# TheMTank/GridUniverse

Measured on AMD Instinct MI355X. Metric: env-steps/sec at N_envs on 32×32 grid, 1/2/4/8 MI355X; bit-exact vs CPU, higher is better.
Workload: dtype int32; 1 GPU; c3: 65536 envs per GPU on the 32x32 generator maze (random.seed(123); np.random.seed(123)), uniform device-RNG actions, auto-reset, 1000 env-steps per launch, int32 (obs,reward,done) rows; envs_per_gpu=65536, env_steps_per_launch=1000, global_envs=65536, parallelism=env-index shards, no data-path collective

## Files before the change

### griduniverse_amd/_lib.py

```python
import ctypes
import os
import re
import subprocess

import numpy as np

_HERE = os.path.dirname(os.path.abspath(__file__))
LIB_PATH = os.environ.get('GU_LIB_PATH') or os.path.join(_HERE, 'lib', 'libgu.so')
CSRC = os.path.join(_HERE, 'csrc')

GU_OK = 0
ERR_NAMES = {-1: 'GU_ERR_INVALID', -2: 'GU_ERR_HIP', -3: 'GU_ERR_NOMEM', -4: 'GU_ERR_STATE',
             -5: 'GU_ERR_COMM', -6: 'GU_ERR_UNSUPPORTED'}

F_AUTO_RESET, F_TRAJECTORY, F_STATS, F_PINNED_IO, F_PACKED = 1, 2, 4, 8, 16
POLICY_UNIFORM, POLICY_STREAM, POLICY_GREEDY, POLICY_SAMPLE = 0, 1, 2, 3
TD_Q_LEARNING, TD_SARSA = 0, 1
NSTEP_MAX = 16
LAMBDA_MAX = 64
REINFORCE_MAX = 1024
IS_MAX = 1024
SEARCH_MAX_M = 64
SEARCH_MAX_D = 256
EXPLORE_MAX_C = 4096
# ... 70 lines not shown
    'gu_read_stats': [_vp, _vp, _vp],
    'gu_get_state': [_vp, _vp, _vp, _vp, _vp],
    'gu_set_state': [_vp, _vp, _vp, _vp, _vp],
    'gu_get_stores': [_vp, _i32, _vp, _vp],
    'gu_done_indices': [_vp, _vp, _vp],
    'gu_look_step_ahead': [_vp, _i64, _vp, _vp, _i32, _vp, _vp, _vp],
    'gu_td_init': [_vp, _f64],
    'gu_td_run': [_vp, _i64, _i32, _f64, _f64, _u32, _u32],
    'gu_td_get_q': [_vp, _i64, _i64, _vp],
    'gu_td_set_q': [_vp, _i64, _i64, _vp],
    'gu_esarsa_run': [_vp, _i64, _f64, _f64, _u32, _u32],
    'gu_double_init': [_vp, _f64],
    'gu_double_run': [_vp, _i64, _f64, _f64, _u32, _u32],
    'gu_double_get_q': [_vp, _i64, _i64, _vp],
    'gu_double_set_q': [_vp, _i64, _i64, _vp],
    'gu_dyna_init': [_vp],
    'gu_dyna_run': [_vp, _i64, _i32, _f64, _f64, _u32, _u32],
    'gu_dyna_get_model': [_vp, _i64, _i64, _vp, _vp, _vp, _vp, _vp],
    'gu_sweep_init': [_vp],
    'gu_sweep_run': [_vp, _i64, _i32, _f64, _f64, _f64, _u32, _u32],
    'gu_sweep_get_queue': [_vp, _i64, _i64, _vp, _vp],
    'gu_diag_sweep_heap': [_vp, _i64, _i64, _vp, _vp],
    'gu_diag_rollout_form': [_vp, _vp, _i32, _vp],
    'gu_search_run': [_vp, _i64, _i32, _i32, _f64, _f64, _u32, _u32, _u32],
    'gu_search_get': [_vp, _i64, _i64, _vp, _vp],
    'gu_explore_init': [_vp],
    'gu_explore_set_tables': [_vp, _i32, _vp, _vp],
    'gu_explore_run': [_vp, _i64, _i32, _f64, _f64, _u32, _u32],
    'gu_explore_get_counts': [_vp, _i64, _i64, _vp],
    'gu_explore_set_counts': [_vp, _i64, _i64, _vp],
    'gu_mcts_init': [_vp, _i32],
    'gu_mcts_set_tables': [_vp, _i32, _vp, _vp, _vp],
    'gu_mcts_run': [_vp, _i64, _i32, _i32, _i32, _f64, _f64, _u32, _u32, _u32],
    'gu_mcts_get': [_vp, _i64, _i64, _vp, _vp, _vp, _vp],
    'gu_mcts_get_tree': [_vp, _i64, _i64, _vp, _vp, _vp, _vp, _vp, _vp],
    'gu_nstep_run': [_vp, _i64, _i32, _i32, _f64, _f64, _u32, _u32],
    'gu_nstep_get_window': [_vp, _i64, _i64, _vp, _vp, _vp],
    'gu_lambda_run': [_vp, _i64, _i32, _i32, _f64, _f64, _f64, _u32, _u32],
    'gu_lambda_get_window': [_vp, _i64, _i64, _vp],
    'gu_ac_init': [_vp, _f64, _f64],
    'gu_ac_run': [_vp, _i64, _f64, _f64, _f64, _u32],
    'gu_ac_get': [_vp, _i64, _i64, _vp, _vp],
    'gu_ac_set': [_vp, _i64, _i64, _vp, _vp],
    'gu_reinforce_run': [_vp, _i64, _i32, _f64, _f64, _f64, _u32],
    'gu_reinforce_get_episode': [_vp, _i64, _i64, _vp, _vp, _vp],
    'gu_is_init': [_vp],
# ... 188 lines not shown
```

### griduniverse_amd/csrc/gu_internal.hpp

```cpp
#pragma once
#include <hip/hip_runtime.h>
#include <stdint.h>
#include <atomic>
#include <string>
#include <vector>

#include "../../include/gu.h"
#include "../../include/gu_diag.h"

#define GU_CELL_OPEN_MASK 0x0Fu
#define GU_CELL_TERM 0x10u
#define GU_CELL_TERM_BIT 4
#define GU_CELL_RPLUS 0x20u
#define GU_CELL_RMINUS 0x40u
#ifndef GU_WIDE_STORE_PAD
#define GU_WIDE_STORE_PAD()                         \
    do {                                            \
        __builtin_amdgcn_sched_barrier(0);          \
        asm volatile("s_nop 1" ::: "memory");       \
        __builtin_amdgcn_sched_barrier(0);          \
    } while (0)
#endif
#define GU_ACTION_OK(raw) ((uint32_t)((int32_t)(raw) + 4) < 8u)
#define GU_CELL_WALL 0x80u
// ... 90 lines not shown
    int32_t overlay_bits = 0;
    uint32_t overlay_param = 0;
    uint32_t overlay_init = 0;
    std::vector<uint8_t> box_flags;
    int32_t fruit_value[3] = {0, 0, 0};
    uint8_t *d_kind = nullptr;
    uint64_t delta_lut = 0;
    int32_t *d_starts = nullptr;
    int32_t *d_nstarts = nullptr;
    int32_t n_starts = 0;
    int32_t start0 = 0;
    int32_t max_starts = 0;
    bool all_single_start = true;
    int32_t n_grids = 1;
    int64_t group = 0;

    int32_t *d_out3 = nullptr;
    uint32_t *d_episode = nullptr;
    int32_t *d_out3_alt = nullptr;
    uint32_t *d_episode_alt = nullptr;
    uint64_t *d_done_bits_alt = nullptr;
    uint32_t *d_nib = nullptr;
    bool nib_valid = false;
    uint32_t *d_tcount = nullptr;
    uint64_t steps_taken = 0;
    int64_t off_lo = 0, off_hi = 0;
    bool off_exact = true;
    uint64_t seed = 0;
    uint32_t seed_prefix = 0;

    int32_t *d_actions = nullptr;
    uint32_t *d_actions_packed = nullptr;
    int64_t actions_T = 0;
    int64_t actions_cap = 0;

    int32_t *d_traj = nullptr;
    int64_t traj_T = 0;
    int traj_kind = 0;
    int traj_written = 0;
    int32_t traj_candidates = 0;
    float traj_probe_ms_best = 0.0f, traj_probe_ms_worst = 0.0f;
    std::vector<float> traj_probe_ms;
    std::vector<uint64_t> traj_probe_addr;
    int32_t traj_kept = -1;
    float traj_search_ms = 0.0f;
    uint64_t traj_peak_bytes = 0;
// ... 334 lines not shown
```

### griduniverse_amd/csrc/gu_kernels.hip

```cpp
#include "gu_overlay.hpp"

#include <cstdio>
#include <cstdlib>

#include <algorithm>
#include <cstring>
#include <vector>

struct ResetArgs {
    int32_t *pos, *done;
    uint32_t *episode;
    const int32_t *starts;
    const uint8_t *mask;
    const int32_t *choice;
    uint64_t *done_bits;
    uint32_t n_starts, seed_prefix, env_id0;
    int64_t N;
    int32_t only_done;
    GridSel gs;
};

__global__ void __launch_bounds__(GU_BLOCK) gu_reset_kernel(const ResetArgs a)
{
    const int64_t e = (int64_t)blockIdx.x * blockDim.x + threadIdx.x;
// ... 329 lines not shown
    pace->bar_num = (uint16_t)gu_opt(h, GU_OPT_PACE_BAR_NUM);
    pace->gain_q = (uint32_t)gu_opt(h, GU_OPT_PACE_GAIN_Q);
    pace->dec_q = (uint32_t)gu_opt(h, GU_OPT_PACE_DEC_Q);
    pace->probe_every = (uint32_t)gu_opt(h, GU_OPT_PACE_PROBE_EVERY);
    pace->adapt = (uint32_t)gu_opt(h, GU_OPT_PACE_ADAPT);
    pace->fixed = 0;
    return GU_OK;
}

int gu_pace_for(gu_engine *h, const GuRolloutPlan &p, int64_t T, GuPaceArgs *pace)
{
    *pace = GuPaceArgs{};
    const int64_t opt = gu_opt(h, GU_OPT_ROLLOUT_PACE);
    if (opt == 0) return GU_OK;
    if (p.pace_eligible && !(opt > 0 && gu_opt(h, GU_OPT_PACE_RECORD) == 0)) {
        GU_TRY(gu_pace_ring_for(h, p.pace_slot, T, p.pace_blocks, p.pace_block, p.row_bytes, pace));
        if (opt > 0) pace->period = (uint32_t)opt, pace->fixed = 1;
        return GU_OK;
    }
    if (opt > 0) pace->period = (uint32_t)opt;
    return GU_OK;
}

__global__ void __launch_bounds__(256) gu_nibble_planes_kernel(const uint8_t *__restrict__ cell, GridSel gs, int32_t W, int32_t H, int32_t dwords, int64_t N,
                                                               uint32_t *__restrict__ out)
{
    const int64_t i = (int64_t)blockIdx.x * blockDim.x + threadIdx.x;
    const int64_t total = ((N + 63) / 64) * dwords * 64;
    if (i >= total) return;
    const int64_t lane = i & 63, j = (i >> 6) % dwords, wave = (i >> 6) / dwords, e = wave * 64 + lane;
    uint32_t word = 0x88888888u;
    if (e < N) {
        const uint8_t *f = cell + (e / gs.group) * gs.grid_stride;
        word = 0;
        for (int32_t k = 0; k < 8; ++k) {
            const int32_t p = (int32_t)j * 8 + k, yp = p / (W + 1), xp = p % (W + 1);
            const bool real = yp >= 1 && yp <= H && xp >= 1;
            const uint32_t b = real ? f[(yp - 1) * W + xp - 1] : GU_CELL_WALL;
            const uint32_t four = ((b >> 5) & 3u) | (((b >> GU_CELL_TERM_BIT) & 1u) << 2) | ((b >> 7) << 3);
            word |= four << (4 * k);
        }
    }
    out[i] = word;
}

int gu_nibble_planes(gu_engine *h)
{
    if (h->nib_valid) return GU_OK;
    const int32_t dwords = gu_nibble_dwords(h);
    const int64_t total = ((h->N + 63) / 64) * dwords * 64;
    if (!h->d_nib) GU_HIP(hipMalloc((void **)&h->d_nib, (size_t)total * sizeof(uint32_t)));
    hipLaunchKernelGGL(gu_nibble_planes_kernel, dim3(gu_blocks(total, 256)), dim3(256), 0, h->stream, h->d_cell, gu_grid_sel(h), h->W, h->H, dwords, h->N, h->d_nib);
    GU_HIP(hipGetLastError());
    h->nib_valid = true;
    return GU_OK;
}

static int gu_rollout_straddles(gu_engine *h, int64_t T, int32_t policy, bool *straddle, uint32_t *epoch_lo)
{
    const bool draws = policy == GU_POLICY_UNIFORM || policy == GU_POLICY_SAMPLE;
    int64_t lo = std::max<int64_t>((int64_t)h->steps_taken + h->off_lo, 0), hi = (int64_t)h->steps_taken + h->off_hi + T - 1;
    if (draws && (lo >> 32) != (hi >> 32) && !h->off_exact) {
        std::vector<int32_t> off((size_t)h->N);
        GU_HIP(hipMemcpyAsync(off.data(), h->d_tcount, (size_t)h->N * 4, hipMemcpyDeviceToHost, h->stream));
        GU_HIP(hipStreamSynchronize(h->stream));
        const auto mm = std::minmax_element(off.begin(), off.end());
        h->off_lo = *mm.first, h->off_hi = *mm.second, h->off_exact = true;
        lo = std::max<int64_t>((int64_t)h->steps_taken + h->off_lo, 0), hi = (int64_t)h->steps_taken + h->off_hi + T - 1;
    }
    *straddle = draws && (lo >> 32) != (hi >> 32);
    *epoch_lo = (uint32_t)(lo >> 32);
    return GU_OK;
}

int gu_launch_rollout(gu_engine *h, int64_t T, int32_t policy, uint32_t flags)
{
    GU_REQUIRE(!(h->overlay && (flags & GU_F_PACKED)), GU_ERR_UNSUPPORTED, "a rollout under %s (gu_set_%s) writes int32 rows only: GU_F_PACKED is refused",
               GU_OVERLAY_NAME[h->overlay], GU_OVERLAY_NAME[h->overlay]);
    GU_REQUIRE(!h->trail_cap || (flags & (GU_F_TRAJECTORY | GU_F_PACKED)), GU_ERR_UNSUPPORTED,
// ... 10 lines not shown
    if (policy == GU_POLICY_SAMPLE)
        hipLaunchKernelGGL(gu_pi_threshold_kernel, dim3(gu_blocks(h->S, 256)), dim3(256), 0, h->stream, h->d_pi[h->vi_cur], h->S, h->d_pi_thr);
    for (bool no_pairs = false; !(p.family == GU_PLAN_KSTEP ? gu_kstep_ensure(h, p) : p.family == GU_PLAN_ROWS ? gu_rows_ensure(h, p, &no_pairs) : true);) {
        exclude |= no_pairs ? GU_PLAN_NO_PAIRS : 1u << p.family;
        p = gu_rollout_plan(h, T, policy, flags, straddle, exclude);
    }

    RolloutArgs a{};
    const int64_t rows = p.traj ? h->traj_T * h->N : 0;
    a.cell = h->d_cell, a.cell_bytes = h->cell_bytes, a.S = h->S, a.W = h->W, a.lut = h->delta_lut, a.gs = gu_grid_sel(h);
    a.greedy = h->d_greedy, a.pi_thr = h->d_pi_thr, a.actions = h->d_actions_packed;
    a.pos = h->pos(), a.reward = h->reward(), a.done = h->done(), a.episode = h->d_episode, a.tcount = h->d_tcount, a.done_bits = h->d_done_bits;
    a.starts = h->d_starts, a.n_starts = (uint32_t)h->n_starts, a.env_id0 = (uint32_t)h->env_id0;
    a.tr_obs = h->d_traj, a.tr_reward = h->d_traj ? h->d_traj + rows : nullptr, a.tr_done = h->d_traj ? h->d_traj + 2 * rows : nullptr;
    a.ret = h->d_ret, a.episodes_fin = h->d_episodes_fin;
    a.N = h->N, a.T = T, a.steps_taken = (uint32_t)h->steps_taken, a.steps_hi = (uint32_t)(h->steps_taken >> 32);
    a.straddle = straddle ? 1 : 0;
    a.seed_prefix0 = h->seed_prefix, a.seed_prefix = straddle ? h->seed_prefix : gu_rng_seed_prefix_epoch(h->seed_prefix, epoch_lo);
    a.gs.per_wave = p.per_wave, a.pi_lds = p.pi_lds, a.stream_lds_off = p.stream_lds_off, a.stream_lds_words = p.stream_lds_words;
    a.half_waves = p.half, a.entry_table = p.entry_table, a.xcd_remap = p.xcd_remap;
    if (p.family == GU_PLAN_ROWS) a.rows = p.table_policy ? h->d_prow : h->d_rows[p.which], a.rows2 = p.pair ? h->d_rows2[p.which] : nullptr, a.row_shift = p.row_shift;
    if (p.family == GU_PLAN_KSTEP) a.rows = h->d_mrows[p.which];
    if (p.need_nib) {
        a.nib = h->d_nib, a.nib_dwords = gu_nibble_dwords(h);
        const uint64_t wp = (uint64_t)(uint16_t)(int16_t)((h->W + 1) * 32), mwp = (uint64_t)(uint16_t)(int16_t)(-(h->W + 1) * 32);
        a.lut_p = mwp | (32ull << 16) | (wp << 32) | ((uint64_t)(uint16_t)(int16_t)-32 << 48);
    }
    if (p.pace_slot >= 0) GU_TRY(gu_pace_for(h, p, T, &a.pace));

    switch (p.family) {
    case GU_PLAN_WIND:
    case GU_PLAN_FRUIT:
    case GU_PLAN_DOORS:
    case GU_PLAN_BOXES: gu_overlay_launch_rollout(h, p, a); break;
    case GU_PLAN_KSTEP: gu_kstep_launch(h, p, a); break;
    case GU_PLAN_ROWS:
        if (!gu_rows_launch(h, p, a)) return gu_fail(GU_ERR_HIP, "gu_rollout_rows_kernel reports static LDS: its table must start at LDS address 0");
        break;
    default: {
        auto launch = policy == GU_POLICY_UNIFORM ? gu_rollout_uniform : policy == GU_POLICY_STREAM ? gu_rollout_stream : policy == GU_POLICY_GREEDY ? gu_rollout_greedy : gu_rollout_sample;
        if (!launch(h, p, a)) {
            p = gu_rollout_plan(h, T, policy, flags, straddle, exclude | GU_PLAN_NO_MAP5);
            a.xcd_remap = p.xcd_remap ? 1 : 0;
            launch(h, p, a);
        }
    }
    }
    GU_HIP(hipGetLastError());
    gu_rollout_plan_form(p, h->rollout_form);
// ... 87 lines not shown
```

### griduniverse_amd/csrc/gu_rollout.hpp

```cpp
#pragma once
#include "gu_map.hpp"
#include "gu_rollout_plan.hpp"

#include <cstdlib>
#include <functional>
#include <type_traits>

__device__ __forceinline__ uint32_t gu_sample_action(uint32_t word, const uint4 q)
{
    return (uint32_t)(word >= q.x) + (uint32_t)(word >= q.y) + (uint32_t)(word >= q.z) - q.w;
}


#define GU_DPP_REDUCE(x, OP)                                                                                     \
    do {                                                                                                         \
        uint32_t o_;                                                                                             \
        o_ = (uint32_t)__builtin_amdgcn_update_dpp(0, (int)(x), 0x111, 0xF, 0xF, false), (x) = OP((x), o_);      \
        o_ = (uint32_t)__builtin_amdgcn_update_dpp(0, (int)(x), 0x112, 0xF, 0xF, false), (x) = OP((x), o_);      \
        o_ = (uint32_t)__builtin_amdgcn_update_dpp(0, (int)(x), 0x114, 0xF, 0xF, false), (x) = OP((x), o_);      \
        o_ = (uint32_t)__builtin_amdgcn_update_dpp(0, (int)(x), 0x118, 0xF, 0xF, false), (x) = OP((x), o_);      \
        o_ = (uint32_t)__builtin_amdgcn_update_dpp(0, (int)(x), 0x142, 0xA, 0xF, false), (x) = OP((x), o_);      \
        o_ = (uint32_t)__builtin_amdgcn_update_dpp(0, (int)(x), 0x143, 0xC, 0xF, false), (x) = OP((x), o_);      \
    } while (0)
#define GU_OP_ADD(a_, b_) ((a_) + (b_))
// ... 282 lines not shown
            step16(word);
        }
    }
    uint32_t q = 0;
    if (TAIL16) {
        for (; i + 16 <= T; i += 16, q += 16) {
            const uint32_t sel = q >> 4;
            step16(sel == 0 ? w[0] : sel == 1 ? w[1] : w[2]);
        }
    }
    for (; i < T; ++i, ++q) {
        const uint32_t sel = q >> 4, word = sel == 0 ? w[0] : sel == 1 ? w[1] : sel == 2 ? w[2] : w[3];
        step1((word >> (2u * (q & 15u))) & 3u);
    }
}

#ifndef GU_STORE_AUX
#define GU_STORE_AUX 18
#endif
#ifndef GU_STORE_AUX_PACKED
#define GU_STORE_AUX_PACKED 16
#endif
typedef uint32_t gu_v3u __attribute__((ext_vector_type(3)));
template <int POLICY, int AUTO, int TRAJ, bool STATS, int MAP>
__global__ void __launch_bounds__(GU_MAX_BLOCK) gu_rollout_kernel(const RolloutArgs a)
{
    constexpr bool LDS = MAP == 1 || MAP == 3;
    extern __shared__ __attribute__((aligned(16))) uint8_t smem[];
    GuPacer pacer;
    pacer.fetch(a.pace, TRAJ == 1 || TRAJ == 3);
    const int64_t e64 = (int64_t)gu_env_block(a.xcd_remap) * blockDim.x + threadIdx.x;
    const bool live = e64 < a.N;
    const uint32_t e = (uint32_t)e64;
    int32_t s = 0, r = 0;
    uint32_t d = 0, ep = 0, tcount0 = 0;
    if (live) {
        s = a.pos[e];
        r = a.reward[e];
        d = (uint32_t)a.done[e];
        ep = a.episode[e];
        tcount0 = a.tcount[e];
    }
    CellMap m = gu_stage_map<LDS>(a.cell, a.cell_bytes, smem, a.gs, MAP == 3 ? 1 : 2);
    const uint32_t nib_region = MAP == 5 ? (threadIdx.x >> 6) * (uint32_t)a.nib_dwords * 256u : 0u;
    if (MAP == 5) {
        const size_t wave = ((size_t)blockIdx.x * blockDim.x + threadIdx.x) >> 6;
        const uint4 *src = reinterpret_cast<const uint4 *>(a.nib + wave * (size_t)a.nib_dwords * 64u);
        uint4 *dst = reinterpret_cast<uint4 *>(smem + nib_region);
        if (wave * 64u < (size_t)a.N)
            for (int32_t i = threadIdx.x & 63; i < a.nib_dwords * 16; i += 64) dst[i] = src[i];
        __syncthreads();
    }
    const uint8_t *greedy = a.greedy;
    if (MAP == 1 && POLICY == GU_POLICY_GREEDY) {
        uint8_t *dst = smem + 2 * a.cell_bytes;
        for (int32_t i = threadIdx.x * 16; i < a.cell_bytes; i += blockDim.x * 16)
            *reinterpret_cast<uint4 *>(dst + i) = *reinterpret_cast<const uint4 *>(a.greedy + i);
        __syncthreads();
        greedy = dst;
    }
    const bool thr_in_lds = MAP == 1 && POLICY == GU_POLICY_SAMPLE && a.pi_lds;
    uint4 *thr_lds = reinterpret_cast<uint4 *>(smem + 2 * a.cell_bytes);
    if (thr_in_lds) {
        for (int32_t i = threadIdx.x; i < a.S; i += blockDim.x) thr_lds[i] = a.pi_thr[i];
        __syncthreads();
    }
    if (!live) return;
    LaneGrid lg = gu_lane_grid<LDS>(a.gs, a.starts, a.n_starts, e, m);

    const uint32_t t_lane = tcount0 + a.steps_taken;
    const uint32_t prefix = gu_rng_prefix(a.seed_prefix, a.env_id0 + e);
    const uint32_t prefix0 = AUTO == 2 ? gu_rng_prefix(a.seed_prefix0, a.env_id0 + e) : prefix;
    const uint32_t epoch0 = (uint32_t)((uint64_t)((int64_t)(((uint64_t)a.steps_hi << 32) | a.steps_taken) + (int64_t)(int32_t)tcount0) >> 32);
    auto prefix_at = [&](uint32_t t) {
        return gu_rng_prefix(gu_rng_seed_prefix_epoch(a.seed_prefix0, epoch0 + (t < t_lane ? 1u : 0u)), a.env_id0 + e);
    };
    constexpr uint32_t TERM5 = 0x20u, TERM5_BIT = 5u;
    auto flags5 = [](uint32_t b) { return (((b >> 5) & 3u) << 3) | (((b >> GU_CELL_TERM_BIT) & 1u) << TERM5_BIT) | ((b >> 7) << 6); };
    uint32_t flags = MAP == 5 ? flags5(m.f[s]) : m.f[s];
    int32_t ret = 0, fin = 0;
    const int32_t W = a.W;
    const uint64_t lut = a.lut;
    const int32_t start0 = lg.starts[0];
    const uint32_t start0_flags = MAP == 5 ? flags5(m.f[start0]) : m.f[start0];
    auto padded = [&](int32_t c) { return (int32_t)(((uint32_t)(c + c / W + W + 2) << 5) + nib_region); };
    int32_t sq = MAP == 5 ? padded(s) : 0;
    const int32_t start0_q = MAP == 5 ? padded(start0) : 0;
    typedef __attribute__((address_space(3))) const uint32_t *lds_word_ptr;
    const uint32_t lane4 = (threadIdx.x & 63u) << 2;
    auto word_at = [&](int32_t cq) { return *(lds_word_ptr)(uintptr_t)(((uint32_t)cq & 0xFFFFFF00u) | lane4); };
    auto four_of = [](uint32_t word, int32_t cq) { return __builtin_amdgcn_ubfe(word, (uint32_t)cq >> 3, 4); };
    auto four_at = [&](int32_t cq) { return four_of(word_at(cq), cq); };
    auto cell5 = [&](int32_t cq) { return four_at(cq) << 3; };
    auto move5 = [&](uint32_t act, int32_t delta, auto &&in_the_shadow) {
        int32_t cand = s + delta;
        asm volatile("" : "+v"(cand));
        const int32_t candq = sq + gu_delta<true>(act, a.lut_p, 0);
        const uint32_t word = word_at(candq);
        in_the_shadow();
        const uint32_t four = four_of(word, candq);
        const bool go = ((flags & TERM5) | four) < 8u;
        s = go ? cand : s;
        sq = go ? candq : sq;
        flags = go ? four << 3 : flags;
    };
    char *po = (char *)a.tr_obs, *pr = (char *)a.tr_reward, *pd = (char *)a.tr_done;
    const char *pa = (const char *)a.actions;
    const uint32_t e4 = e * 4u;
    const int64_t row = a.N * 4;
    const uint32_t row32 = (uint32_t)row;
    const int64_t trow = TRAJ == 3 ? a.N * 12 : row;
    const uint32_t trow32 = (uint32_t)trow;
    const uint32_t te = TRAJ == 3 ? e * 12u : e4;
    __amdgpu_buffer_rsrc_t ro = __builtin_amdgcn_make_buffer_rsrc(po, 0, 0xFFFFFFFFu, 0x00020000);
    __amdgpu_buffer_rsrc_t rr = __builtin_amdgcn_make_buffer_rsrc(pr, 0, 0xFFFFFFFFu, 0x00020000);
    __amdgpu_buffer_rsrc_t rd = __builtin_amdgcn_make_buffer_rsrc(pd, 0, 0xFFFFFFFFu, 0x00020000);
    auto emit = [&](int32_t s_, int32_t r_, uint32_t d_, uint32_t soff) {
        if (TRAJ == 1) {
            __builtin_amdgcn_raw_buffer_store_b32(s_, ro, e4, soff, GU_STORE_AUX);
            __builtin_amdgcn_raw_buffer_store_b32(r_, rr, e4, soff, GU_STORE_AUX);
            __builtin_amdgcn_raw_buffer_store_b32((int32_t)d_, rd, e4, soff, GU_STORE_AUX);
        } else if (TRAJ == 2) {
            __builtin_amdgcn_raw_buffer_store_b32((int32_t)((uint32_t)s_ | (((uint32_t)r_ & 0xFFu) << 16) | (d_ << 24)), ro, e4, soff, GU_STORE_AUX_PACKED);
        } else if (TRAJ == 3) {
            const gu_v3u triple = {(uint32_t)s_, (uint32_t)r_, d_};
            __builtin_amdgcn_raw_buffer_store_b96(triple, ro, te, soff, GU_STORE_AUX);
            GU_WIDE_STORE_PAD();
        }
    };
    bool held = false;
    int32_t held_s = 0, held_r = 0;
    uint32_t held_d = 0, held_soff = 0;
    auto release = [&]() {
        if (MAP == 5 && TRAJ && held) emit(held_s, held_r, held_d, held_soff);
        held = false;
    };
    auto rebase = [&](int64_t rows) {
        release();
        po += rows * trow;
        ro = __builtin_amdgcn_make_buffer_rsrc(po, 0, 0xFFFFFFFFu, 0x00020000);
        if (TRAJ == 1) {
            pr += rows * trow;
            pd += rows * trow;
            rr = __builtin_amdgcn_make_buffer_rsrc(pr, 0, 0xFFFFFFFFu, 0x00020000);
            rd = __builtin_amdgcn_make_buffer_rsrc(pd, 0, 0xFFFFFFFFu, 0x00020000);
        }
    };

    if (AUTO == 1 && MAP != 5) flags = (flags & ~GU_CELL_TERM) | (d << GU_CELL_TERM_BIT);

    auto step = [&](uint32_t act, uint32_t soff) {
        const int32_t delta = gu_delta<MAP != 0>(act, lut, W);
        if (AUTO == 1) {
            const bool was_done = MAP == 5 ? d != 0u : (flags & GU_CELL_TERM) != 0u;
            ep += was_done;
            s = was_done ? start0 : s;
            flags = was_done ? start0_flags : flags;
            if (MAP == 5) sq = was_done ? start0_q : sq;
        } else if (AUTO == 2) {
            if (d) {
                s = lg.starts[gu_rng_start_index(prefix0, ep, lg.n_starts)];
                ++ep;
                if (MAP == 5) sq = padded(s);
                flags = MAP == 5 ? cell5(sq) : m.f[s];
            }
        }
        if (MAP == 5) {
            move5(act, delta, [&]() {
                if (TRAJ && held) {
                    __builtin_amdgcn_sched_barrier(0);
                    emit(held_s, held_r, held_d, held_soff);
                    __builtin_amdgcn_sched_barrier(0);
                }
            });
        } else {
            s = gu_move(s, flags, act, delta);
            flags = m.f[s];
        }
        r = MAP == 5 ? __builtin_amdgcn_sbfe((int32_t)0xF6F60AFFu, flags, 8) : (MAP >= 2) ? gu_reward_packed(flags) : (int32_t)m.r[s];
        d = __builtin_amdgcn_ubfe(flags, MAP == 5 ? TERM5_BIT : GU_CELL_TERM_BIT, 1);
        if (STATS) {
            ret += r;
            fin += (int32_t)d;
        }
        if (MAP == 5 && TRAJ) held = true, held_s = s, held_r = r, held_d = d, held_soff = soff;
        else emit(s, r, d, soff);
    };
    auto step1 = [&](uint32_t act) {
        step(act, 0);
        if (TRAJ) rebase(1);
    };

    pacer.start(a.pace, TRAJ == 1 || TRAJ == 3);
    if (POLICY == GU_POLICY_UNIFORM && a.straddle) {
        uint32_t t = t_lane;
#pragma nounroll
        for (int64_t i = 0; i < a.T; ++i, ++t) step1((gu_rng_word(prefix_at(t), GU_RNG_STREAM_ACTION, t >> 4) >> (2u * (t & 15u))) & 3u);
    } else if (POLICY == GU_POLICY_UNIFORM) {
        const uint32_t t_first = __builtin_amdgcn_readfirstlane(t_lane);
        if (__all(t_lane == t_first)) {
            uint32_t t = t_first;
            int64_t i = 0;
            if (t & 15u) {
                const uint32_t word = gu_rng_word(prefix, GU_RNG_STREAM_ACTION, t >> 4);
                for (; i < a.T && (t & 7u); ++i, ++t) step1((word >> (2u * (t & 15u))) & 3u);
                if ((t & 15u) == 8u && i + 8 <= a.T) {
#pragma unroll
                    for (uint32_t j = 0; j < 8; ++j) step(__builtin_amdgcn_ubfe(word, 16 + 2 * j, 2), j * trow32);
                    if (TRAJ) rebase(8);
                    i += 8, t += 8;
                }
                for (; i < a.T && (t & 15u); ++i, ++t) step1((word >> (2u * (t & 15u))) & 3u);
                pacer.after((uint32_t)i);
            }
            for (; i + 16 <= a.T; i += 16, t += 16) {
                uint32_t word = gu_rng_word(prefix, GU_RNG_STREAM_ACTION, t >> 4);
                if (MAP == 5) asm volatile("" : "+v"(word));
#pragma unroll
                for (uint32_t j = 0; j < 16; ++j) step(__builtin_amdgcn_ubfe(word, 2 * j, 2), j * trow32);
                if (TRAJ) rebase(16);
                if (i + 16 < a.T) pacer.after(16);
            }
            if (i < a.T) {
                const uint32_t word = gu_rng_word(prefix, GU_RNG_STREAM_ACTION, t >> 4);
                uint32_t j = 0;
                if (i + 8 <= a.T) {
#pragma unroll
                    for (uint32_t k = 0; k < 8; ++k) step(__builtin_amdgcn_ubfe(word, 2 * k, 2), k * trow32);
                    if (TRAJ) rebase(8);
                    i += 8, j = 8;
                }
                for (; i < a.T; ++i, ++j) step1((word >> (2u * j)) & 3u);
            }
        } else {
            uint32_t t = t_lane;
            uint32_t word = gu_rng_word(prefix, GU_RNG_STREAM_ACTION, t >> 4);
            for (int64_t i = 0; i < a.T; ++i) {
                step1((word >> (2u * (t & 15u))) & 3u);
                ++t;
                if ((t & 15u) == 0u) word = gu_rng_word(prefix, GU_RNG_STREAM_ACTION, t >> 4);
// ... 144 lines not shown
{
    static std::atomic<uint64_t> raised{0};
    gu_allow_lds(KERN, raised, h->device, lds, (size_t)h->lds_per_cu);
    if (BASE_ZERO) {
        static std::atomic<int> base_zero{0};
        if (!base_zero.load(std::memory_order_relaxed)) {
            hipFuncAttributes fa{};
            const bool got = hipFuncGetAttributes(&fa, (const void *)KERN) == hipSuccess;
            base_zero.store(got && fa.sharedSizeBytes == 0 ? 1 : 2, std::memory_order_relaxed);
        }
        if (base_zero.load(std::memory_order_relaxed) != 1) return false;
    }
    hipLaunchKernelGGL(KERN, dim3(blocks), dim3(block), lds, h->stream, args...);
    return true;
}

template <int POLICY>
static bool gu_rollout_general(gu_engine *h, const GuRolloutPlan &p, const RolloutArgs &a)
{
    bool ok = false;
    gu_pick<2, 1, 0>(p.auto_mode, [&](auto auto_c) {
        gu_pick<0, 3, 2, 1>(p.traj, [&](auto traj_c) {
            gu_pick<0, 1>(p.stats, [&](auto stats_c) {
                gu_pick<0, 5, 3, 1>(p.map, [&](auto map_c) {
                    constexpr int AUTO = decltype(auto_c)::value, TRAJ = decltype(traj_c)::value, MAP = decltype(map_c)::value;
                    constexpr bool STATS = decltype(stats_c)::value != 0;
                    if constexpr (MAP < 3 || POLICY == GU_POLICY_UNIFORM || POLICY == GU_POLICY_STREAM)
                        ok = gu_lds_launch<gu_rollout_kernel<POLICY, AUTO, TRAJ, STATS, MAP>, MAP == 5>(h, p.blocks, p.block, p.lds, a);
                });
            });
        });
    });
    return ok;
}

bool gu_rollout_uniform(gu_engine *h, const GuRolloutPlan &p, const RolloutArgs &a);
bool gu_rollout_stream(gu_engine *h, const GuRolloutPlan &p, const RolloutArgs &a);
bool gu_rollout_greedy(gu_engine *h, const GuRolloutPlan &p, const RolloutArgs &a);
bool gu_rollout_sample(gu_engine *h, const GuRolloutPlan &p, const RolloutArgs &a);
bool gu_rows_ensure(gu_engine *h, const GuRolloutPlan &p, bool *no_pairs);
bool gu_rows_launch(gu_engine *h, const GuRolloutPlan &p, const RolloutArgs &a);
bool gu_kstep_ensure(gu_engine *h, const GuRolloutPlan &p);
void gu_kstep_launch(gu_engine *h, const GuRolloutPlan &p, const RolloutArgs &a);
int gu_nibble_planes(gu_engine *h);
int gu_pace_for(gu_engine *h, const GuRolloutPlan &p, int64_t T, GuPaceArgs *pace);
```

### griduniverse_amd/engine.py

```python
import ctypes

import numpy as np

from . import _lib
from ._lib import check, ptr
from .grid import GridSpec, check_sense_args

_POLICIES = {'uniform': _lib.POLICY_UNIFORM, 'stream': _lib.POLICY_STREAM, 'greedy': _lib.POLICY_GREEDY,
             'sample': _lib.POLICY_SAMPLE}
_EXPLORE_RULES = {'ucb': _lib.EXPLORE_UCB, 'thompson': _lib.EXPLORE_THOMPSON, 0: _lib.EXPLORE_UCB, 1: _lib.EXPLORE_THOMPSON}
_TD_METHODS = {'q_learning': _lib.TD_Q_LEARNING, 'sarsa': _lib.TD_SARSA, 0: _lib.TD_Q_LEARNING, 1: _lib.TD_SARSA}


def _learner_flags(trajectory, stats):
    return (_lib.F_TRAJECTORY if trajectory else 0) | (_lib.F_STATS if stats else 0)


def _tables(x, row, name, dtype=np.float64):
    x = np.asarray(x, dtype)
    x = _lib.as_array(x.reshape((-1,) + row) if x.ndim == len(row) else x, dtype, None, name)
    if x.ndim != len(row) + 1 or x.shape[1:] != row:
        raise ValueError('{} must have shape (n, {}), got {}'.format(name, ', '.join(str(k) for k in row), x.shape))
    return x

# ... 248 lines not shown
        ms = ctypes.c_float(0.0)
        check(self.lib.gu_probe_trajectory(self._h, ctypes.byref(ms)))
        return ms.value

    def rollout(self, T, policy='uniform', auto_reset=True, trajectory=True, stats=False):
        tflag = _lib.F_PACKED if trajectory == 'packed' else (_lib.F_TRAJECTORY if trajectory else 0)
        flags = (_lib.F_AUTO_RESET if auto_reset else 0) | tflag | (_lib.F_STATS if stats else 0)
        check(self.lib.gu_rollout(self._h, int(T), _POLICIES[policy], flags))

    ROLLOUT_FORM = ('family', 'layout', 'map', 'block', 'workgroups', 'lds_bytes', 'flags', 'K', 'row_shift', 'stream_words', 'pace_slot', 'pace_mode')
    ROLLOUT_FAMILIES = {0: None, 1: 'general', 2: 'rows', 3: 'kstep', 4: 'wind', 5: 'fruit', 6: 'doors', 7: 'boxes'}
    ROLLOUT_FLAG_BITS = ('pair', 'half', 'per_wave', 'pi_lds', 'straddle', 'entry_table', 'xcd_remap')

    def rollout_last_form(self):
        words = np.zeros(len(self.ROLLOUT_FORM), np.int32)
        n = ctypes.c_int32(0)
        check(self.lib.gu_diag_rollout_form(self._h, ptr(words), words.size, ctypes.byref(n)))
        out = dict(zip(self.ROLLOUT_FORM, (int(w) for w in words)))
        out.update((name, bool(out['flags'] >> bit & 1)) for bit, name in enumerate(self.ROLLOUT_FLAG_BITS))
        out['family'] = self.ROLLOUT_FAMILIES[out['family']]
        out['words'] = [int(w) for w in words]
        return out

    def calibrate_rollout(self, T, policy='uniform', auto_reset=True, trajectory=True, stats=False):
        flags = (_lib.F_AUTO_RESET if auto_reset else 0) | (_lib.F_STATS if stats else 0)
        flags |= _lib.F_PACKED if trajectory == 'packed' else (_lib.F_TRAJECTORY if trajectory else 0)
        check(self.lib.gu_rollout_calibrate(self._h, int(T), _POLICIES[policy], flags))

    def rollout_pacing_totals(self):
        ms = ctypes.c_float(0.0)
        n = [ctypes.c_int32(0) for _ in range(4)]
        check(self.lib.gu_rollout_pacing_totals(self._h, ctypes.byref(ms), *[ctypes.byref(x) for x in n]))
        return dict(calibration_ms=ms.value, launches_spent=n[0].value, kinds_paced=n[1].value, kinds_from_cache=n[2].value, kinds_waiting=n[3].value)

    def rollout_pacing(self, policy='uniform', auto_reset=True, packed=False):
        period, n = ctypes.c_int32(0), ctypes.c_int32(0)
        a, b, c = ctypes.c_float(0.0), ctypes.c_float(0.0), ctypes.c_float(0.0)
        rc = self.lib.gu_rollout_pacing(self._h, _POLICIES[policy], (_lib.F_AUTO_RESET if auto_reset else 0) | (_lib.F_PACKED if packed else 0), ctypes.byref(period),
                                        ctypes.byref(a), ctypes.byref(b), ctypes.byref(n), ctypes.byref(c))
        if rc == -4:
            return None
        check(rc)
        return dict(period=period.value, ms_unpaced=a.value, ms_paced=b.value, evaluated=n.value, calibration_ms=c.value)

    def rollout_pace_log(self, policy='uniform', auto_reset=True, packed=False):
        buf = np.zeros((61, 8), dtype=np.uint64)
# ... 573 lines not shown
```

### include/gu.h

```cpp
#ifndef GU_H
#define GU_H

#include <stddef.h>
#include <stdint.h>

#ifdef __cplusplus
extern "C" {
#endif

#define GU_ABI_VERSION 1

#define GU_OK 0
#define GU_ERR_INVALID (-1)
#define GU_ERR_HIP (-2)
#define GU_ERR_NOMEM (-3)
#define GU_ERR_STATE (-4)
#define GU_ERR_COMM (-5)
#define GU_ERR_UNSUPPORTED (-6)

#define GU_F_AUTO_RESET 1u
#define GU_F_TRAJECTORY 2u
#define GU_F_STATS 4u
#define GU_F_PACKED 16u
#define GU_F_PINNED_IO 8u
// ... 119 lines not shown
int gu_done_indices(gu_handle h, int32_t *idx, int32_t *count);

int gu_td_init(gu_handle h, double q0);
int gu_td_run(gu_handle h, int64_t T, int32_t method, double alpha, double gamma, uint32_t eps_q16, uint32_t flags);
int gu_td_get_q(gu_handle h, int64_t env0, int64_t n, double *q);
int gu_td_set_q(gu_handle h, int64_t env0, int64_t n, const double *q);

int gu_esarsa_run(gu_handle h, int64_t T, double alpha, double gamma, uint32_t eps_q16, uint32_t flags);

int gu_double_init(gu_handle h, double q0);
int gu_double_run(gu_handle h, int64_t T, double alpha, double gamma, uint32_t eps_q16, uint32_t flags);
int gu_double_get_q(gu_handle h, int64_t env0, int64_t n, double *q);
int gu_double_set_q(gu_handle h, int64_t env0, int64_t n, const double *q);

int gu_dyna_init(gu_handle h);
int gu_dyna_run(gu_handle h, int64_t T, int32_t P, double alpha, double gamma, uint32_t eps_q16, uint32_t flags);
int gu_dyna_get_model(gu_handle h, int64_t env0, int64_t n, int32_t *next, int32_t *reward, int32_t *done, int32_t *list, int32_t *count);

int gu_sweep_init(gu_handle h);
int gu_sweep_run(gu_handle h, int64_t T, int32_t P, double theta, double alpha, double gamma, uint32_t eps_q16, uint32_t flags);
int gu_sweep_get_queue(gu_handle h, int64_t env0, int64_t n, uint64_t *key, int32_t *size);
int gu_diag_sweep_heap(gu_handle h, int64_t env0, int64_t n, uint64_t *heap, int32_t *pos);
int gu_diag_rollout_form(gu_handle h, int32_t *form, int32_t capacity, int32_t *count);

#define GU_SEARCH_MAX_M 64
#define GU_SEARCH_MAX_D 256
int gu_search_run(gu_handle h, int64_t T, int32_t M, int32_t D, double alpha, double gamma, uint32_t eps_q16, uint32_t eps_sim_q16,
                  uint32_t flags);
int gu_search_get(gu_handle h, int64_t env0, int64_t n, double *score, int64_t *sim_steps);

#define GU_EXPLORE_MAX_C 4096
#define GU_EXPLORE_COUNT_MAX 0x3FFFFFFFu
int gu_explore_init(gu_handle h);
int gu_explore_set_tables(gu_handle h, int32_t C, const double *U, const double *B);
int gu_explore_run(gu_handle h, int64_t T, int32_t mode, double alpha, double gamma, uint32_t eps_q16, uint32_t flags);
int gu_explore_get_counts(gu_handle h, int64_t env0, int64_t n, uint32_t *counts);
int gu_explore_set_counts(gu_handle h, int64_t env0, int64_t n, const uint32_t *counts);

#define GU_MCTS_MAX_SIMS 255
#define GU_MCTS_MAX_DEPTH 64
int gu_mcts_init(gu_handle h, int32_t max_sims);
int gu_mcts_set_tables(gu_handle h, int32_t C, const double *U, const double *B, const double *I);
int gu_mcts_run(gu_handle h, int64_t T, int32_t M, int32_t H, int32_t D, double alpha, double gamma, uint32_t eps_q16, uint32_t eps_sim_q16,
                uint32_t flags);
int gu_mcts_get(gu_handle h, int64_t env0, int64_t n, double *w, uint32_t *visits, int32_t *nodes, int64_t *sim_steps);
int gu_mcts_get_tree(gu_handle h, int64_t env0, int64_t n, int32_t *state, int32_t *parent, int32_t *child, uint32_t *visits, double *w,
// ... 86 lines not shown
```

Measured before the change: 615.9 billion env-steps/s.

## Pack maze cells into 2-bit planes when grid has only plain cell kinds

Adds a 2-bit-per-cell encoding of the per-wave LDS grid plane, used when a device-side check finds that every cell falls into one of four classes (open, wall, terminal +reward, terminal -reward). This halves the LDS footprint and the staging traffic, and could allow more waves per CU. The per-step move test and reward extraction switch to bitfield lookups, and staging now goes through direct global-to-LDS loads. The detection adds a one-time host sync and a second planes kernel launch.

```diff
diff --git a/griduniverse_amd/_lib.py b/griduniverse_amd/_lib.py
--- a/griduniverse_amd/_lib.py
+++ b/griduniverse_amd/_lib.py
@@ -116,6 +116,7 @@
     'gu_sweep_get_queue': [_vp, _i64, _i64, _vp, _vp],
     'gu_diag_sweep_heap': [_vp, _i64, _i64, _vp, _vp],
     'gu_diag_rollout_form': [_vp, _vp, _i32, _vp],
+    'gu_diag_nibble_bits': [_vp],
     'gu_search_run': [_vp, _i64, _i32, _i32, _f64, _f64, _u32, _u32, _u32],
     'gu_search_get': [_vp, _i64, _i64, _vp, _vp],
     'gu_explore_init': [_vp],
diff --git a/griduniverse_amd/csrc/gu_internal.hpp b/griduniverse_amd/csrc/gu_internal.hpp
--- a/griduniverse_amd/csrc/gu_internal.hpp
+++ b/griduniverse_amd/csrc/gu_internal.hpp
@@ -136,6 +136,7 @@
     uint64_t *d_done_bits_alt = nullptr;
     uint32_t *d_nib = nullptr;
     bool nib_valid = false;
+    int32_t nib_bits = 0;
     uint32_t *d_tcount = nullptr;
     uint64_t steps_taken = 0;
     int64_t off_lo = 0, off_hi = 0;
diff --git a/griduniverse_amd/csrc/gu_kernels.hip b/griduniverse_amd/csrc/gu_kernels.hip
--- a/griduniverse_amd/csrc/gu_kernels.hip
+++ b/griduniverse_amd/csrc/gu_kernels.hip
@@ -375,39 +375,75 @@
     return GU_OK;
 }
 
+template <int BITS>
 __global__ void __launch_bounds__(256) gu_nibble_planes_kernel(const uint8_t *__restrict__ cell, GridSel gs, int32_t W, int32_t H, int32_t dwords, int64_t N,
-                                                               uint32_t *__restrict__ out)
-{
+                                                               uint32_t *__restrict__ out, uint32_t *__restrict__ not_plain, const uint8_t *__restrict__ kind,
+                                                               int32_t kind_stride, const int32_t *__restrict__ starts)
+{
+    constexpr int32_t PER = 32 / BITS;
     const int64_t i = (int64_t)blockIdx.x * blockDim.x + threadIdx.x;
     const int64_t total = ((N + 63) / 64) * dwords * 64;
     if (i >= total) return;
     const int64_t lane = i & 63, j = (i >> 6) % dwords, wave = (i >> 6) / dwords, e = wave * 64 + lane;
-    uint32_t word = 0x88888888u;
+    uint32_t word = BITS == 4 ? 0x88888888u : 0u;
     if (e < N) {
         const uint8_t *f = cell + (e / gs.group) * gs.grid_stride;
+        bool odd = false;
         word = 0;
-        for (int32_t k = 0; k < 8; ++k) {
-            const int32_t p = (int32_t)j * 8 + k, yp = p / (W + 1), xp = p % (W + 1);
+        for (int32_t k = 0; k < PER; ++k) {
+            const int32_t p = (int32_t)j * PER + k, yp = p / (W + 1), xp = p % (W + 1);
             const bool real = yp >= 1 && yp <= H && xp >= 1;
             const uint32_t b = real ? f[(yp - 1) * W + xp - 1] : GU_CELL_WALL;
             const uint32_t four = ((b >> 5) & 3u) | (((b >> GU_CELL_TERM_BIT) & 1u) << 2) | ((b >> 7) << 3);
-            word |= four << (4 * k);
-        }
+            if (BITS == 4) {
+                word |= four << (4 * k);
+                odd |= !(four == 0u || (four >= 5u && four <= 8u));
+                if (real && kind) odd |= kind[(e / gs.group) * kind_stride + (yp - 1) * W + xp - 1] == 3 && (b & GU_CELL_RMINUS);
+            } else {
+                word |= gu_two_of_four(four) << (2 * k);
+            }
+        }
+        if (BITS == 4 && j == 0) {
+            const int64_t g = e / gs.group;
+            for (int32_t k = 0; k < gs.n_starts[g]; ++k) odd |= (f[starts[g * gs.max_starts + k]] & GU_CELL_WALL) != 0u;
+        }
+        if (BITS == 4 && odd) atomicOr(not_plain, 1u);
     }
     out[i] = word;
 }
+
+static inline int32_t gu_two_bit_dwords(const gu_engine *h) { return (((gu_nibble_cells(h) + 15) / 16) + 3) & ~3; }
 
 int gu_nibble_planes(gu_engine *h)
 {
     if (h->nib_valid) return GU_OK;
     const int32_t dwords = gu_nibble_dwords(h);
-    const int64_t total = ((h->N + 63) / 64) * dwords * 64;
-    if (!h->d_nib) GU_HIP(hipMalloc((void **)&h->d_nib, (size_t)total * sizeof(uint32_t)));
-    hipLaunchKernelGGL(gu_nibble_planes_kernel, dim3(gu_blocks(total, 256)), dim3(256), 0, h->stream, h->d_cell, gu_grid_sel(h), h->W, h->H, dwords, h->N, h->d_nib);
-    GU_HIP(hipGetLastError());
+    const int64_t waves = (h->N + 63) / 64, total = waves * dwords * 64;
+    if (!h->d_nib) GU_HIP(hipMalloc((void **)&h->d_nib, (size_t)(total + 1) * sizeof(uint32_t)));
+    uint32_t *not_plain = h->d_nib + total;
+    GU_HIP(hipMemsetAsync(not_plain, 0, sizeof(uint32_t), h->stream));
+    hipLaunchKernelGGL(gu_nibble_planes_kernel<4>, dim3(gu_blocks(total, 256)), dim3(256), 0, h->stream, h->d_cell, gu_grid_sel(h), h->W, h->H, dwords, h->N, h->d_nib,
+                       not_plain, h->d_kind, h->cell_bytes, h->d_starts);
+    GU_HIP(hipGetLastError());
+    h->nib_bits = 4;
+#ifndef GU_NIB_FORCE4
+    uint32_t odd = 1;
+    GU_HIP(hipMemcpyAsync(&odd, not_plain, sizeof odd, hipMemcpyDeviceToHost, h->stream));
+    GU_HIP(hipStreamSynchronize(h->stream));
+    if (!odd) {
+        const int32_t dwords2 = gu_two_bit_dwords(h);
+        const int64_t total2 = waves * dwords2 * 64;
+        hipLaunchKernelGGL(gu_nibble_planes_kernel<2>, dim3(gu_blocks(total2, 256)), dim3(256), 0, h->stream, h->d_cell, gu_grid_sel(h), h->W, h->H, dwords2, h->N,
+                           h->d_nib, not_plain, nullptr, 0, nullptr);
+        GU_HIP(hipGetLastError());
+        h->nib_bits = 2;
+    }
+#endif
     h->nib_valid = true;
     return GU_OK;
 }
+
+int gu_diag_nibble_bits(gu_handle h) { return h && h->nib_valid ? h->nib_bits : 0; }
 
 static int gu_rollout_straddles(gu_engine *h, int64_t T, int32_t policy, bool *straddle, uint32_t *epoch_lo)
 {
@@ -464,9 +500,11 @@
     if (p.family == GU_PLAN_ROWS) a.rows = p.table_policy ? h->d_prow : h->d_rows[p.which], a.rows2 = p.pair ? h->d_rows2[p.which] : nullptr, a.row_shift = p.row_shift;
     if (p.family == GU_PLAN_KSTEP) a.rows = h->d_mrows[p.which];
     if (p.need_nib) {
-        a.nib = h->d_nib, a.nib_dwords = gu_nibble_dwords(h);
-        const uint64_t wp = (uint64_t)(uint16_t)(int16_t)((h->W + 1) * 32), mwp = (uint64_t)(uint16_t)(int16_t)(-(h->W + 1) * 32);
-        a.lut_p = mwp | (32ull << 16) | (wp << 32) | ((uint64_t)(uint16_t)(int16_t)-32 << 48);
+        const bool two = h->nib_bits == 2;
+        a.nib = h->d_nib, a.nib_dwords = two ? gu_two_bit_dwords(h) : gu_nibble_dwords(h);
+        const int32_t one = two ? 16 : 32;
+        const uint64_t wp = (uint64_t)(uint16_t)(int16_t)((h->W + 1) * one), mwp = (uint64_t)(uint16_t)(int16_t)(-(h->W + 1) * one);
+        a.lut_p = mwp | ((uint64_t)one << 16) | (wp << 32) | ((uint64_t)(uint16_t)(int16_t)-one << 48);
     }
     if (p.pace_slot >= 0) GU_TRY(gu_pace_for(h, p, T, &a.pace));
 
diff --git a/griduniverse_amd/csrc/gu_rollout.hpp b/griduniverse_amd/csrc/gu_rollout.hpp
--- a/griduniverse_amd/csrc/gu_rollout.hpp
+++ b/griduniverse_amd/csrc/gu_rollout.hpp
@@ -328,10 +328,12 @@
 #define GU_STORE_AUX_PACKED 16
 #endif
 typedef uint32_t gu_v3u __attribute__((ext_vector_type(3)));
+__host__ __device__ __forceinline__ uint32_t gu_two_of_four(uint32_t four) { return (four & 8u) ? 0u : (four & 4u) ? ((four & 2u) ? 3u : 2u) : 1u; }
 template <int POLICY, int AUTO, int TRAJ, bool STATS, int MAP>
 __global__ void __launch_bounds__(GU_MAX_BLOCK) gu_rollout_kernel(const RolloutArgs a)
 {
     constexpr bool LDS = MAP == 1 || MAP == 3;
+    constexpr bool NIB = MAP == 5 || MAP == 6, TWO = MAP == 6;
     extern __shared__ __attribute__((aligned(16))) uint8_t smem[];
     GuPacer pacer;
     pacer.fetch(a.pace, TRAJ == 1 || TRAJ == 3);
@@ -348,13 +350,14 @@
         tcount0 = a.tcount[e];
     }
     CellMap m = gu_stage_map<LDS>(a.cell, a.cell_bytes, smem, a.gs, MAP == 3 ? 1 : 2);
-    const uint32_t nib_region = MAP == 5 ? (threadIdx.x >> 6) * (uint32_t)a.nib_dwords * 256u : 0u;
-    if (MAP == 5) {
+    const uint32_t nib_region = NIB ? (threadIdx.x >> 6) * (uint32_t)a.nib_dwords * 256u : 0u;
+    if (NIB) {
+        typedef __attribute__((address_space(3))) void *lds_void_ptr;
         const size_t wave = ((size_t)blockIdx.x * blockDim.x + threadIdx.x) >> 6;
-        const uint4 *src = reinterpret_cast<const uint4 *>(a.nib + wave * (size_t)a.nib_dwords * 64u);
-        uint4 *dst = reinterpret_cast<uint4 *>(smem + nib_region);
+        const uint32_t *src = a.nib + wave * (size_t)a.nib_dwords * 64u + (threadIdx.x & 63u) * 4u;
+        const uint32_t base = __builtin_amdgcn_readfirstlane(nib_region);
         if (wave * 64u < (size_t)a.N)
-            for (int32_t i = threadIdx.x & 63; i < a.nib_dwords * 16; i += 64) dst[i] = src[i];
+            for (int32_t k = 0; k < a.nib_dwords; k += 4) __builtin_amdgcn_global_load_lds(src + k * 64, (lds_void_ptr)(uintptr_t)(base + (uint32_t)k * 256u), 16, 0, 0);
         __syncthreads();
     }
     const uint8_t *greedy = a.greedy;
@@ -381,21 +384,25 @@
     auto prefix_at = [&](uint32_t t) {
         return gu_rng_prefix(gu_rng_seed_prefix_epoch(a.seed_prefix0, epoch0 + (t < t_lane ? 1u : 0u)), a.env_id0 + e);
     };
-    constexpr uint32_t TERM5 = 0x20u, TERM5_BIT = 5u;
-    auto flags5 = [](uint32_t b) { return (((b >> 5) & 3u) << 3) | (((b >> GU_CELL_TERM_BIT) & 1u) << TERM5_BIT) | ((b >> 7) << 6); };
-    uint32_t flags = MAP == 5 ? flags5(m.f[s]) : m.f[s];
+    constexpr uint32_t TERM5_BIT = TWO ? 4u : 5u, TERM5 = 1u << TERM5_BIT;
+    auto flags5 = [](uint32_t b) {
+        if (TWO) return gu_two_of_four(((b >> 5) & 3u) | (((b >> GU_CELL_TERM_BIT) & 1u) << 2) | ((b >> 7) << 3)) << 3;
+        return (((b >> 5) & 3u) << 3) | (((b >> GU_CELL_TERM_BIT) & 1u) << TERM5_BIT) | ((b >> 7) << 6);
+    };
+    uint32_t flags = NIB ? flags5(m.f[s]) : m.f[s];
     int32_t ret = 0, fin = 0;
     const int32_t W = a.W;
     const uint64_t lut = a.lut;
     const int32_t start0 = lg.starts[0];
-    const uint32_t start0_flags = MAP == 5 ? flags5(m.f[start0]) : m.f[start0];
-    auto padded = [&](int32_t c) { return (int32_t)(((uint32_t)(c + c / W + W + 2) << 5) + nib_region); };
-    int32_t sq = MAP == 5 ? padded(s) : 0;
-    const int32_t start0_q = MAP == 5 ? padded(start0) : 0;
+    const uint32_t start0_flags = NIB ? flags5(m.f[start0]) : m.f[start0];
+    constexpr uint32_t CELL_SHIFT = TWO ? 4u : 5u, CELL_BITS = TWO ? 2u : 4u;
+    auto padded = [&](int32_t c) { return (int32_t)(((uint32_t)(c + c / W + W + 2) << CELL_SHIFT) + nib_region); };
+    int32_t sq = NIB ? padded(s) : 0;
+    const int32_t start0_q = NIB ? padded(start0) : 0;
     typedef __attribute__((address_space(3))) const uint32_t *lds_word_ptr;
     const uint32_t lane4 = (threadIdx.x & 63u) << 2;
     auto word_at = [&](int32_t cq) { return *(lds_word_ptr)(uintptr_t)(((uint32_t)cq & 0xFFFFFF00u) | lane4); };
-    auto four_of = [](uint32_t word, int32_t cq) { return __builtin_amdgcn_ubfe(word, (uint32_t)cq >> 3, 4); };
+    auto four_of = [](uint32_t word, int32_t cq) { return __builtin_amdgcn_ubfe(word, (uint32_t)cq >> 3, CELL_BITS); };
     auto four_at = [&](int32_t cq) { return four_of(word_at(cq), cq); };
     auto cell5 = [&](int32_t cq) { return four_at(cq) << 3; };
     auto move5 = [&](uint32_t act, int32_t delta, auto &&in_the_shadow) {
@@ -405,7 +412,7 @@
         const uint32_t word = word_at(candq);
         in_the_shadow();
         const uint32_t four = four_of(word, candq);
-        const bool go = ((flags & TERM5) | four) < 8u;
+        const bool go = TWO ? __builtin_amdgcn_ubfe(0x00000101u, flags, four) != 0u : ((flags & TERM5) | four) < 8u;
         s = go ? cand : s;
         sq = go ? candq : sq;
         flags = go ? four << 3 : flags;
@@ -438,7 +445,7 @@
     int32_t held_s = 0, held_r = 0;
     uint32_t held_d = 0, held_soff = 0;
     auto release = [&]() {
-        if (MAP == 5 && TRAJ && held) emit(held_s, held_r, held_d, held_soff);
+        if (NIB && TRAJ && held) emit(held_s, held_r, held_d, held_soff);
         held = false;
     };
     auto rebase = [&](int64_t rows) {
@@ -453,25 +460,25 @@
         }
     };
 
-    if (AUTO == 1 && MAP != 5) flags = (flags & ~GU_CELL_TERM) | (d << GU_CELL_TERM_BIT);
+    if (AUTO == 1 && !NIB) flags = (flags & ~GU_CELL_TERM) | (d << GU_CELL_TERM_BIT);
 
     auto step = [&](uint32_t act, uint32_t soff) {
         const int32_t delta = gu_delta<MAP != 0>(act, lut, W);
         if (AUTO == 1) {
-            const bool was_done = MAP == 5 ? d != 0u : (flags & GU_CELL_TERM) != 0u;
+            const bool was_done = NIB ? d != 0u : (flags & GU_CELL_TERM) != 0u;
             ep += was_done;
             s = was_done ? start0 : s;
             flags = was_done ? start0_flags : flags;
-            if (MAP == 5) sq = was_done ? start0_q : sq;
+            if (NIB) sq = was_done ? start0_q : sq;
         } else if (AUTO == 2) {
             if (d) {
                 s = lg.starts[gu_rng_start_index(prefix0, ep, lg.n_starts)];
                 ++ep;
-                if (MAP == 5) sq = padded(s);
-                flags = MAP == 5 ? cell5(sq) : m.f[s];
-            }
-        }
-        if (MAP == 5) {
+                if (NIB) sq = padded(s);
+                flags = NIB ? cell5(sq) : m.f[s];
+            }
+        }
+        if (NIB) {
             move5(act, delta, [&]() {
                 if (TRAJ && held) {
                     __builtin_amdgcn_sched_barrier(0);
@@ -483,13 +490,13 @@
             s = gu_move(s, flags, act, delta);
             flags = m.f[s];
         }
-        r = MAP == 5 ? __builtin_amdgcn_sbfe((int32_t)0xF6F60AFFu, flags, 8) : (MAP >= 2) ? gu_reward_packed(flags) : (int32_t)m.r[s];
-        d = __builtin_amdgcn_ubfe(flags, MAP == 5 ? TERM5_BIT : GU_CELL_TERM_BIT, 1);
+        r = NIB ? __builtin_amdgcn_sbfe((int32_t)(TWO ? 0xF60AFFFFu : 0xF6F60AFFu), flags, 8) : (MAP >= 2) ? gu_reward_packed(flags) : (int32_t)m.r[s];
+        d = __builtin_amdgcn_ubfe(flags, NIB ? TERM5_BIT : GU_CELL_TERM_BIT, 1);
         if (STATS) {
             ret += r;
             fin += (int32_t)d;
         }
-        if (MAP == 5 && TRAJ) held = true, held_s = s, held_r = r, held_d = d, held_soff = soff;
+        if (NIB && TRAJ) held = true, held_s = s, held_r = r, held_d = d, held_soff = soff;
         else emit(s, r, d, soff);
     };
     auto step1 = [&](uint32_t act) {
@@ -521,7 +528,7 @@
             }
             for (; i + 16 <= a.T; i += 16, t += 16) {
                 uint32_t word = gu_rng_word(prefix, GU_RNG_STREAM_ACTION, t >> 4);
-                if (MAP == 5) asm volatile("" : "+v"(word));
+                if (NIB) asm volatile("" : "+v"(word));
 #pragma unroll
                 for (uint32_t j = 0; j < 16; ++j) step(__builtin_amdgcn_ubfe(word, 2 * j, 2), j * trow32);
                 if (TRAJ) rebase(16);
@@ -712,11 +719,11 @@
     gu_pick<2, 1, 0>(p.auto_mode, [&](auto auto_c) {
         gu_pick<0, 3, 2, 1>(p.traj, [&](auto traj_c) {
             gu_pick<0, 1>(p.stats, [&](auto stats_c) {
-                gu_pick<0, 5, 3, 1>(p.map, [&](auto map_c) {
+                gu_pick<6, 0, 5, 3, 1>(p.map == 5 && h->nib_bits == 2 ? 6 : p.map, [&](auto map_c) {
                     constexpr int AUTO = decltype(auto_c)::value, TRAJ = decltype(traj_c)::value, MAP = decltype(map_c)::value;
                     constexpr bool STATS = decltype(stats_c)::value != 0;
                     if constexpr (MAP < 3 || POLICY == GU_POLICY_UNIFORM || POLICY == GU_POLICY_STREAM)
-                        ok = gu_lds_launch<gu_rollout_kernel<POLICY, AUTO, TRAJ, STATS, MAP>, MAP == 5>(h, p.blocks, p.block, p.lds, a);
+                        ok = gu_lds_launch<gu_rollout_kernel<POLICY, AUTO, TRAJ, STATS, MAP>, MAP == 5 || MAP == 6>(h, p.blocks, p.block, p.lds, a);
                 });
             });
         });
diff --git a/griduniverse_amd/engine.py b/griduniverse_amd/engine.py
--- a/griduniverse_amd/engine.py
+++ b/griduniverse_amd/engine.py
@@ -294,6 +294,9 @@
         out['words'] = [int(w) for w in words]
         return out
 
+    def nibble_bits(self):
+        return int(self.lib.gu_diag_nibble_bits(self._h))
+
     def calibrate_rollout(self, T, policy='uniform', auto_reset=True, trajectory=True, stats=False):
         flags = (_lib.F_AUTO_RESET if auto_reset else 0) | (_lib.F_STATS if stats else 0)
         flags |= _lib.F_PACKED if trajectory == 'packed' else (_lib.F_TRAJECTORY if trajectory else 0)
diff --git a/include/gu.h b/include/gu.h
--- a/include/gu.h
+++ b/include/gu.h
@@ -165,6 +165,7 @@
 int gu_sweep_get_queue(gu_handle h, int64_t env0, int64_t n, uint64_t *key, int32_t *size);
 int gu_diag_sweep_heap(gu_handle h, int64_t env0, int64_t n, uint64_t *heap, int32_t *pos);
 int gu_diag_rollout_form(gu_handle h, int32_t *form, int32_t capacity, int32_t *count);
+int gu_diag_nibble_bits(gu_handle h);
 
 #define GU_SEARCH_MAX_M 64
 #define GU_SEARCH_MAX_D 256
```

Measured after the change: 615.3 billion env-steps/s. About the same (-0.1%).
